# 2InfinityN6eyond/AbsoluteTrack

Hardware: AMD Instinct MI355X
Metric: hand-frames/sec (higher is better)
Workload: dtype f32 (backbone products as two fp16 pieces per operand, fp32 accumulation); 1 GPU; 4 fisheye cameras x 2 hands per frame, 2 views per hand, 96x96 crops, known-skeleton path, full hot path (resample+backbone+head+FK) + all-gather of records; frames_per_gpu=1024, src_image=480x636 u8 x 4 cameras, parallelism=frame-shard x1, world=1, backend=none (single process), outputs_finite=True

## Files before the change

### absolutetrack_amd/csrc/conv_w4.hip

```cpp
#include <type_traits>

#include "ut_kernels.h"
#include "ut_conv_dev.h"

namespace ut {
namespace {

constexpr int W4_WPIX = 288;
constexpr int W4_MI = 9;
constexpr int W4_NLOAD = 9;
constexpr int W4_NSTG = 5;
constexpr int W4_DIST = 2;
constexpr int W4_NSET = W4_DIST + 1;
constexpr unsigned W4_HOOB = 0x80000000u;
static_assert(9 % W4_NSET == 0, "the register sets of the weight fragments line up across slices");
constexpr int w4_cap(int pixels, int wi, int hi) { return ((pixels / (wi * hi)) * (hi + 1) * (wi + 1) + 2 * (wi + 2) + 15) / 16 * 16; }

template <int WI, int HI, int SCH, int WPX, bool S2 = false, bool CHAIN = false>
__global__ __launch_bounds__(256, 1) void conv_w4_kernel(typename std::conditional<CHAIN, W4ChainLaunch, ConvLaunch>::type p, int tiles_n, int n_tiles) {
  extern __shared__ __attribute__((aligned(16))) char smem[];
  constexpr int MI = W4_MI, PW = WI + 1, PH = HI + 1, HW = WI * HI;
  static_assert(!S2 || (SCH == 32 && WPX == 1), "phase planes: two 16-channel planes per buffer, four 32-channel blocks per tile");
  static_assert(!(S2 && CHAIN), "chains: the stride-1 forms");
  constexpr int LDAUX = CHAIN ? 16 : 0;
  constexpr int BM = W4_WPIX * WPX;
  constexpr int NCB = 4 / WPX, BN = 32 * NCB;
  constexpr int NG = SCH / 4, NHG = NG / 2;
  constexpr int KS = 9 * SCH / 16;
  constexpr int NBUF = SCH == 32 ? 2 : 3;
  constexpr int AHEAD = NBUF - 1;
  constexpr int RP = 256 / NG;
  constexpr int CAP = w4_cap(BM, WI, HI);
  constexpr int GSTRIDE = CAP * 16;
  constexpr int STAGE = NG * GSTRIDE;
  constexpr int SLOT = NBUF * STAGE;
  constexpr int KTAB = SLOT + 16;
  constexpr int EPI = SLOT + (CHAIN ? 64 : 16);
  static_assert(BM % HW == 0, "a tile is a whole number of maps: every tile has the same padded layout");
  static_assert(BM * NG == W4_NLOAD * 256 && KS % W4_NSET == 0 && (SCH == 32 || SCH == 16) && (WPX == 1 || WPX == 2), "shape");
  static_assert((NG - 2) * GSTRIDE + (2 * PW + 2) * 16 < 65536, "fragment reads: everything but the lane's base fits the immediate offset");

  const int tid = threadIdx.x;
  const int lane = tid & 63;
  const int wave = __builtin_amdgcn_readfirstlane(tid >> 6);
  const int wm = WPX == 1 ? 0 : wave >> 1;
  const int wco = WPX == 1 ? wave : wave & 1;
  const int fr = lane & 31, fh = lane >> 5;

  const int M = p.n_img * HW;
  int n_slices = (!S2 && p.k_cin > 0 ? p.k_cin : p.cin) / (S2 ? 16 : SCH);
  const int n_chunks = p.k_pad / 32;

  __amdgpu_buffer_rsrc_t a_rsrc = __builtin_amdgcn_make_buffer_rsrc(
      const_cast<float*>(p.in), 0, (int)((size_t)M * (S2 ? 4 : 1) * p.cin * sizeof(float)), 0x00020000);
  __amdgpu_buffer_rsrc_t w_rsrc = __builtin_amdgcn_make_buffer_rsrc(
      const_cast<void*>(p.w_split), 0, (int)((size_t)(p.cout_pad / 32) * n_chunks * 4096), 0x00020000);
  __amdgpu_buffer_rsrc_t r_rsrc = __builtin_amdgcn_make_buffer_rsrc(
      const_cast<float*>(p.res ? p.res : p.bias), 0, p.res ? (int)((size_t)M * p.cout_store * sizeof(float)) : 0, 0x00020000);
  __amdgpu_buffer_rsrc_t o_rsrc =
      __builtin_amdgcn_make_buffer_rsrc(p.out, 0, (int)((size_t)M * p.cout_store * sizeof(float)), 0x00020000);
  const __amdgpu_buffer_rsrc_t q_rsrc = __builtin_amdgcn_make_buffer_rsrc(p.tile_counter, 0, 4, 0x00020000);

  float x_scale = 1.f, x_unscale = 1.f;
  if (p.in_max) {
    bool ok, adapted;
    split_act_scale(p.in_max, p.in_obs, p.split_adaptive, x_scale, x_unscale, ok, adapted);
    split_scale_report(ok, adapted, p.status, p.adapt_count);
  }
  float tot_unscale = p.split_unscale * x_unscale;
  float floor_v = p.relu ? 0.f : -__builtin_huge_valf();
  const float* bias_c = p.bias;
  unsigned* out_max_c = p.out_max;
  int guard_k = 0;
  bool guarded = false;
  float xs_n = x_scale;
  __amdgpu_buffer_rsrc_t a_rsrc_n = a_rsrc, w_rsrc_n = w_rsrc;
  int n_slices_n = n_slices;
  const unsigned row_b = (unsigned)p.cout_store * 4u;

  const int grid = gridDim.x;
  int slot = blockIdx.x;
  if ((grid & 7) == 0) slot = (blockIdx.x & 7) * (grid >> 3) + (blockIdx.x >> 3);

  unsigned h_wa[W4_NLOAD], pb[MI];
#pragma unroll
  for (int j = 0; j < W4_NLOAD; ++j) {
    const int k = RP * j + tid / NG, img = k / HW, rem = k - img * HW, y = rem / WI, x = rem - y * WI;
    h_wa[j] = (unsigned)((PW + 1 + img * (PH * PW) + y * PW + x) * 16 + ((tid % NG) >> 1) * GSTRIDE + (tid & 1) * 8);
  }
#pragma unroll
  for (int i = 0; i < MI; ++i) {
    const int k = wm * W4_WPIX + 32 * i + fr, img = k / HW, rem = k - img * HW, y = rem / WI, x = rem - y * WI;
    pb[i] = (unsigned)((img * (PH * PW) + y * PW + x) * 16 + fh * GSTRIDE);
  }
  const unsigned h_step = (unsigned)(RP * p.cin) * 4u;
#define W4_H_BASE(TILE) ((unsigned)((((TILE) / tiles_n) * BM + tid / NG) * p.cin + 4 * (tid % NG)) * 4u)
#define W4_H_BASE_U(UNIT) ((unsigned)(((UNIT) * BM + tid / NG) * p.cin + 4 * (tid % NG)) * 4u)
  unsigned h_in[S2 ? W4_NLOAD : 1], po_a = 0, po_b = 0, pb1[S2 ? MI : 1];
  if constexpr (S2) {
#pragma unroll
    for (int j = 0; j < W4_NLOAD; ++j) {
      const int k = RP * j + tid / NG, img = k / HW, rem = k - img * HW, y = rem / WI, x = rem - y * WI;
      h_in[j] = (unsigned)(((img * 2 * HI + 2 * y) * 2 * WI + 2 * x) * p.cin + 4 * (tid & 3)) * 4u;
    }
    const bool second = (tid & 4) != 0;
    po_a = second ? 0u : (unsigned)((2 * WI + 1) * p.cin) * 4u;
    po_b = second ? (unsigned)(2 * WI * p.cin) * 4u : (unsigned)p.cin * 4u;
#pragma unroll
    for (int i = 0; i < MI; ++i) pb1[i] = pb[i] + (unsigned)STAGE;
  }
#define W4S_BASE(TILE) ((unsigned)(((TILE) / tiles_n) * (BM * 4)) * (unsigned)p.cin * 4u)

  f32x16 acc[MI];
  u32x4 xp[MI][2];
  u32x4 wf[W4_NSET][2];
  float4 stg[S2 ? W4_NLOAD : W4_NSTG];
  const unsigned w_lane = (unsigned)lane * 16u;

#define W4_READ_X(I, PC, S, TAP, BASE)                                                               \
  xp[I][PC] = *reinterpret_cast<const u32x4*>(smem + (BASE)[I] + (unsigned)(((PC) * NHG + (SCH == 32 ? 2 * (S) : 0)) * GSTRIDE + (((TAP) / 3) * PW + (TAP) % 3) * 16));
#define W4_LOAD_W_OF(RS, SET, PL, CH, S, WROW)                                                       \
  {                                                                                                  \
    const unsigned so_ = (WROW) + (unsigned)((wco * n_chunks + (CH)) * 4096 + ((S) * 2 + (PL)) * 1024); \
    wf[SET][PL] = __builtin_bit_cast(u32x4, __builtin_amdgcn_raw_buffer_load_b128(RS, w_lane, so_, 0)); \
  }
#define W4_LOAD_W(SET, PL, CH, S, WROW) W4_LOAD_W_OF(w_rsrc, SET, PL, CH, S, WROW)
#define W4S_PLANE(Q) ((0x190 >> (Q)) & 1)
#define W4S_TAPP(Q) ((int)((0x414344310ull >> (4 * (Q))) & 15))
#define W4S_TAPO(Q) ((int)((0x715348620ull >> (4 * (Q))) & 15))
#define W4S_BASEOF(Q) ((Q) >= 5 ? pb1 : pb)
#define W4_TAP(Q) (SCH == 32 ? (Q) >> 1 : (Q))
#define W4_CHUNK(SL, Q) (SCH == 32 ? (SL) * 9 + ((Q) >> 1) : ((SL) >> 1) * 9 + (Q))
#define W4_HALF(SL, Q) (SCH == 32 ? (Q) & 1 : (SL) & 1)
#define W4_MFMA(WSET, N)                                                                             \
  {                                                                                                  \
    constexpr int pr_ = (N) / MI, i_ = (N) % MI;                                                     \
    constexpr int wp_ = pr_ == 1 ? 1 : 0, xq_ = pr_ == 0 ? 1 : 0;       \
    acc[i_] = __builtin_amdgcn_mfma_f32_32x32x16_f16(__builtin_bit_cast(f16x8, xp[i_][xq_]),         \
                                                     __builtin_bit_cast(f16x8, wf[WSET][wp_]), acc[i_], 0, 0, 0);  \
  }
#define W4_PIN() { __builtin_amdgcn_sched_barrier(0); asm volatile("" ::: "memory"); __builtin_amdgcn_sched_barrier(0); }
#define W4_ROW_OFF(I, R) ((unsigned)((I) * 32 + 8 * ((R) >> 2) + ((R) & 3)) * row_bs)
#define W4_SPLIT_STORE(V, WA)                                                                        \
  {                                                                                                  \
    unsigned a0_, b0_, a1_, b1_;                                                                     \
    split_pair_scaled((V).x, (V).y, x_scale, a0_, b0_);                                              \
    split_pair_scaled((V).z, (V).w, x_scale, a1_, b1_);                                              \
    *reinterpret_cast<u32x2*>(smem + (WA)) = u32x2{a0_, a1_};                                        \
    *reinterpret_cast<u32x2*>(smem + (WA) + NHG * GSTRIDE) = u32x2{b0_, b1_};                        \
  }

  int tile = slot;
  int next_tile = 0;
  int cur_buf = 0;
  unsigned out_bits = 0;
  const unsigned slot_addr = (unsigned)(unsigned long)(lds_char*)smem + (unsigned)SLOT;
  const int tn_sh = tiles_n == 2 ? 1 : 0, tn_mask = tiles_n - 1;
  int u_c = slot, s_c = 0, u_o = -1, s_o = 0, nx_u = -1, nx_s = 0, adv_u = -1, adv_s = 0, k_c = 0, k_n = 0;
  bool dep = false;
  int steps = 0;
  if constexpr (CHAIN) {
    steps = p.n_layers << tn_sh;
    u_o = grid + slot < n_tiles ? grid + slot : -1;
    if (tid < p.n_layers) {
      const unsigned bits = *p.lay[tid].in_max;
      const int e = (int)(bits >> 23);
      float sc_, un_;
      *reinterpret_cast<int*>(smem + KTAB + 4 * tid) = split_pow2_for(e, bits == 0u || e == 255, sc_, un_);
      if (tid > 0 && e == 255 && blockIdx.x == 0 && p.status) atomicOr(p.status, UT_SPLIT_RANGE);
    }
  }

  for (int k = tid; k < NBUF * STAGE / 16; k += 256) *reinterpret_cast<u32x4*>(smem + k * 16) = u32x4{0, 0, 0, 0};
  __syncthreads();
  unsigned h_base = S2 ? 0u : CHAIN ? W4_H_BASE_U(slot) : W4_H_BASE(tile);
  unsigned w_row = CHAIN ? 0u : (unsigned)((tile % tiles_n) * NCB) * (unsigned)n_chunks * 4096u;
  unsigned w_row_next = w_row;
  if constexpr (CHAIN) k_c = k_n = slot_read(slot_addr + (unsigned)(KTAB - SLOT));
  if constexpr (!S2) {
#pragma unroll
    for (int a = 0; a < AHEAD; ++a)
#pragma unroll
      for (int j = 0; j < W4_NLOAD; ++j) {
        const float4 v = __builtin_bit_cast(float4, __builtin_amdgcn_raw_buffer_load_b128(a_rsrc, h_base + (unsigned)j * h_step, (unsigned)(a * SCH * 4), LDAUX));
        if (a == AHEAD - 1 && KS == 9 && j >= W4_NLOAD - 4) stg[j % W4_NSTG] = v;
        else W4_SPLIT_STORE(v, (unsigned)(a * STAGE) + h_wa[j])
      }
#pragma unroll
    for (int g = 0; g < W4_DIST; ++g) { W4_LOAD_W(g, 0, W4_CHUNK(0, g), W4_HALF(0, g), w_row) W4_LOAD_W(g, 1, W4_CHUNK(0, g), W4_HALF(0, g), w_row) }
  } else {
    const unsigned t0 = W4S_BASE(tile);
#pragma unroll
    for (int j = 0; j < W4_NLOAD; ++j) {
      const float4 v = __builtin_bit_cast(float4, __builtin_amdgcn_raw_buffer_load_b128(a_rsrc, h_in[j] + po_a + t0, 0, 0));
      W4_SPLIT_STORE(v, h_wa[j])
    }
#pragma unroll
    for (int j = 0; j < W4_NLOAD; ++j) {
      const float4 v = __builtin_bit_cast(float4, __builtin_amdgcn_raw_buffer_load_b128(a_rsrc, h_in[j] + po_b + t0, 0, 0));
      if (j == 0) W4_SPLIT_STORE(v, (unsigned)STAGE + h_wa[j])
      else stg[j] = v;
    }
#pragma unroll
    for (int g = 0; g < W4_DIST; ++g) { W4_LOAD_W(g, 0, W4S_TAPO(g), 0, w_row) W4_LOAD_W(g, 1, W4S_TAPO(g), 0, w_row) }
  }
  __syncthreads();
#pragma unroll
  for (int i = 0; i < MI; ++i) {
    W4_READ_X(i, 1, 0, 0, pb)
    if (i < MI - 1) { W4_READ_X(i, 0, 0, 0, pb) }
  }

#define W4_SLOT_BODY(N)                                                                              \
        {                                                                                            \
          if ((N) == 0 && q != KS - 1) { W4_READ_X(MI - 1, 0, W4_HALF(sl, q), W4_TAP(q), rb) }       \
          if ((N) >= 1 && (N) <= 9 && q1 < KS) { W4_READ_X(((N) + 8) % 9, 1, W4_HALF(sl, q1), W4_TAP(q1), rb) } \
          if ((N) >= 1 && (N) <= 9 && q1 == KS) { W4_READ_X(((N) + 8) % 9, 1, 0, 0, nb) }            \
          if ((N) >= 19 && (N) <= 26 && q1 < KS) { W4_READ_X(((N) + 8) % 9, 0, W4_HALF(sl, q1), W4_TAP(q1), rb) } \
          if ((N) >= 19 && (N) <= 26 && q1 == KS) { W4_READ_X(((N) + 8) % 9, 0, 0, 0, nb) }          \
          if (((N) == 10 || (N) == 11) && qd < KS) { W4_LOAD_W(qd % W4_NSET, (N) & 1, W4_CHUNK(sl, qd), W4_HALF(sl, qd), w_row) } \
          if (((N) == 10 || (N) == 11) && qd >= KS) { W4_LOAD_W_OF(wr_after, qd % W4_NSET, (N) & 1, W4_CHUNK(sl_after, qd - KS), W4_HALF(sl_after, qd - KS), row_after) } \
          if ((N) == 12 && q >= 4 && q < 4 + W4_NLOAD) { const float4 v_ = stg[(q + W4_NSTG - 4) % W4_NSTG]; split_pair_scaled(v_.x, v_.y, xs_f, cv0, cv1); } \
          if ((N) == 13 && q >= 4 && q < 4 + W4_NLOAD) {                                             \
            const float4 v_ = stg[(q + W4_NSTG - 4) % W4_NSTG];                                      \
            unsigned a1_, b1_;                                                                       \
            split_pair_scaled(v_.z, v_.w, xs_f, a1_, b1_);                                           \
            *reinterpret_cast<u32x2*>(smem + wbuf + h_wa[(q + 5) % 9]) = u32x2{cv0, a1_};            \
            *reinterpret_cast<u32x2*>(smem + wbuf + h_wa[(q + 5) % 9] + NHG * GSTRIDE) = u32x2{cv1, b1_}; \
          }                                                                                          \
          if (KS == 9 && (N) == 12 && q < 4) { const float4 v_ = stg[q % W4_NSTG]; split_pair_scaled(v_.x, v_.y, xs_p, cv0, cv1); } \
          if (KS == 9 && (N) == 13 && q < 4) {       \
            const float4 v_ = stg[q % W4_NSTG];                                                      \
            unsigned a1_, b1_;                                                                       \
            split_pair_scaled(v_.z, v_.w, xs_p, a1_, b1_);                                           \
            *reinterpret_cast<u32x2*>(smem + pbuf + h_wa[q + 5]) = u32x2{cv0, a1_};                  \
            *reinterpret_cast<u32x2*>(smem + pbuf + h_wa[q + 5] + NHG * GSTRIDE) = u32x2{cv1, b1_};  \
          }                                                                                          \
          if ((N) == 14 && q < W4_NLOAD)                                                             \
            stg[q % W4_NSTG] = __builtin_bit_cast(float4, __builtin_amdgcn_raw_buffer_load_b128(f_rsrc, h_base + (unsigned)q * h_step, f_soff, LDAUX)); \
          if ((N) == 16 && q == KS / 2 && sl == 0 && tid == 0) *reinterpret_cast<int*>(smem + SLOT) = (CHAIN ? 2 * grid : grid) + ticket; \
          W4_PIN();                                                                                  \
          W4_MFMA(ws, N);                                                                            \
          W4_PIN();                                                                                  \
        }
#define W4_SLICE()                                                                                   \
      _Pragma("clang loop unroll(full)") for (int q = 0; q < KS; ++q) {                              \
        const int ws = q % W4_NSET;                                                                  \
        unsigned cv0 = 0, cv1 = 0;      \
         \
        const int q1 = q + 1, qd = q + W4_DIST;                                                      \
        if (q == KS - 1) {                                                                           \
                                       \
          W4_READ_X(MI - 1, 0, W4_HALF(sl, KS - 1), 8, rb)                                           \
                                                                            \
          if (CHAIN && sl == 0) asm volatile("s_waitcnt vmcnt(0)" ::: "memory");                     \
          asm volatile("s_waitcnt lgkmcnt(0)" ::: "memory");                                         \
          __builtin_amdgcn_s_barrier();                                                              \
          asm volatile("" ::: "memory");                                                             \
          if constexpr (CHAIN) {                                                                     \
            if (sl == 0) { W4_CHAIN_NEXT() }                                                         \
          } else if (sl == 0) {                                                                      \
            next_tile = slot_read(slot_addr);                                                        \
            w_row_next = (unsigned)((next_tile % tiles_n) * NCB) * (unsigned)n_chunks * 4096u;       \
          }                                                                                          \
        }                                                                                            \
        W4_SLOT_BODY(0) W4_SLOT_BODY(1) W4_SLOT_BODY(2) W4_SLOT_BODY(3) W4_SLOT_BODY(4) W4_SLOT_BODY(5) W4_SLOT_BODY(6) W4_SLOT_BODY(7) W4_SLOT_BODY(8) \
        W4_SLOT_BODY(9) W4_SLOT_BODY(10) W4_SLOT_BODY(11) W4_SLOT_BODY(12) W4_SLOT_BODY(13) W4_SLOT_BODY(14) W4_SLOT_BODY(15) W4_SLOT_BODY(16) W4_SLOT_BODY(17) \
        W4_SLOT_BODY(18) W4_SLOT_BODY(19) W4_SLOT_BODY(20) W4_SLOT_BODY(21) W4_SLOT_BODY(22) W4_SLOT_BODY(23) W4_SLOT_BODY(24) W4_SLOT_BODY(25) W4_SLOT_BODY(26) \
      }

#define W4S_CV_N(Q) ((Q) == 4 ? 3 : (Q) == 8 ? 1 : 2)
#define W4S_CV_J(Q, NN) ((Q) < 4 ? 2 * (Q) + 1 + (NN) : (Q) == 4 ? (NN) : (Q) < 8 ? 2 * (Q) - 7 + (NN) : 0)
#define W4S_CV_DST(Q) (((Q) < 4 || (Q) == 8) ? (unsigned)STAGE : 0u)
#define W4S_LD_N(Q) ((Q) == 0 ? 3 : (Q) == 4 ? 1 : 2)
#define W4S_LD_J(Q, NN) ((Q) == 0 ? (NN) : (Q) < 4 ? 2 * (Q) + 1 + (NN) : (Q) == 4 ? 0 : 2 * (Q) - 9 + (NN))
#define W4S_SLOT_BODY(N)                                                                             \
        {                                                                                            \
          if ((N) == 0) { W4_READ_X(MI - 1, 0, W4S_PLANE(q), W4S_TAPP(q), W4S_BASEOF(q)) }          \
          if ((N) == 9 && (q == 4 || q == 8)) {                                                      \
                                         \
            asm volatile("s_waitcnt lgkmcnt(0)" ::: "memory");                                       \
            __builtin_amdgcn_s_barrier();                                                            \
            asm volatile("" ::: "memory");                                                           \
            if (q == 8 && sl == 0) {                                                                 \
              next_tile = slot_read(slot_addr);                                                      \
              w_row_next = (unsigned)((next_tile % tiles_n) * NCB) * (unsigned)n_chunks * 4096u;     \
            }                                                                                        \
          }                                                                                          \
          if ((N) >= 1 && (N) <= 9 && q != 4 && q != 8) { W4_READ_X(((N) + 8) % 9, 1, W4S_PLANE(q1), W4S_TAPP(q1), W4S_BASEOF(q1)) } \
          if ((N) >= 10 && (N) <= 18 && (q == 4 || q == 8)) { W4_READ_X(((N) + 8) % 9, 1, W4S_PLANE(q1), W4S_TAPP(q1), W4S_BASEOF(q1)) } \
          if ((N) >= 19 && (N) <= 26) { W4_READ_X(((N) + 8) % 9, 0, W4S_PLANE(q1), W4S_TAPP(q1), W4S_BASEOF(q1)) } \
          if (((N) == 10 || (N) == 11) && qd < 9) { W4_LOAD_W(qd % W4_NSET, (N) & 1, (sl >> 1) * 9 + W4S_TAPO(qd), sl & 1, w_row) } \
          if (((N) == 10 || (N) == 11) && qd >= 9) { W4_LOAD_W(qd % W4_NSET, (N) & 1, (sl_after >> 1) * 9 + W4S_TAPO(qd - 9), sl_after & 1, row_after) } \
           \
          if ((N) >= 10 && (N) <= 21 && ((N) - 10) / 4 < W4S_CV_N(q)) {                              \
            const float4 v_ = stg[W4S_CV_J(q, ((N) - 10) / 4) % 9];                                  \
            constexpr int part_ = ((N) - 10) & 3;                                                    \
            if (part_ == 0 || part_ == 2) {                                                          \
              const f16x2 h_ = __builtin_bit_cast(f16x2, __builtin_amdgcn_cvt_pkrtz((part_ ? v_.z : v_.x) * x_scale, (part_ ? v_.w : v_.y) * x_scale)); \
              (part_ ? cvh1 : cvh0) = __builtin_bit_cast(unsigned, h_);                              \
              cvf = (float)h_[0];                                                                    \
            } else {                                                                                 \
              const f16x2 h_ = __builtin_bit_cast(f16x2, part_ == 1 ? cvh0 : cvh1);                  \
              const float ra_ = __builtin_fmaf(part_ == 1 ? v_.x : v_.z, x_scale, -cvf);             \
              const float rb_ = __builtin_fmaf(part_ == 1 ? v_.y : v_.w, x_scale, -(float)h_[1]);    \
              const unsigned p_ = __builtin_bit_cast(unsigned, __builtin_amdgcn_cvt_pkrtz(ra_, rb_)); \
              if (part_ == 1) cvp0 = p_;                                                             \
              else {                                                                                 \
                *reinterpret_cast<u32x2*>(smem + W4S_CV_DST(q) + h_wa[W4S_CV_J(q, ((N) - 10) / 4) % 9]) = u32x2{cvh0, cvh1}; \
                *reinterpret_cast<u32x2*>(smem + W4S_CV_DST(q) + h_wa[W4S_CV_J(q, ((N) - 10) / 4) % 9] + NHG * GSTRIDE) = u32x2{cvp0, p_}; \
              }                                                                                      \
            }                                                                                        \
          }                                                                                          \
          if ((N) >= 22 && (N) <= 24 && (N) - 22 < W4S_LD_N(q))                                      \
            stg[W4S_LD_J(q, (N) - 22) % 9] = __builtin_bit_cast(float4, __builtin_amdgcn_raw_buffer_load_b128(    \
                a_rsrc, h_in[W4S_LD_J(q, (N) - 22) % 9] + (q < 4 ? hb_a : hb_b), f_soff, 0));        \
          if ((N) == 16 && q == 1 && sl == 0 && tid == 0) *reinterpret_cast<int*>(smem + SLOT) = grid + ticket; \
          W4_PIN();                                                                                  \
          W4_MFMA(ws, N);                                                                            \
          W4_PIN();                                                                                  \
        }
#define W4S_SLICE()                                                                                  \
      _Pragma("clang loop unroll(full)") for (int q = 0; q < 9; ++q) {                               \
        const int ws = q % W4_NSET;                                                                  \
        unsigned cvh0 = 0, cvh1 = 0, cvp0 = 0;                       \
        float cvf = 0.f;                                                                             \
        const int q1 = (q + 1) % 9, qd = q + W4_DIST;                                                \
        W4S_SLOT_BODY(0) W4S_SLOT_BODY(1) W4S_SLOT_BODY(2) W4S_SLOT_BODY(3) W4S_SLOT_BODY(4) W4S_SLOT_BODY(5) W4S_SLOT_BODY(6) W4S_SLOT_BODY(7) W4S_SLOT_BODY(8) \
        W4S_SLOT_BODY(9) W4S_SLOT_BODY(10) W4S_SLOT_BODY(11) W4S_SLOT_BODY(12) W4S_SLOT_BODY(13) W4S_SLOT_BODY(14) W4S_SLOT_BODY(15) W4S_SLOT_BODY(16) W4S_SLOT_BODY(17) \
        W4S_SLOT_BODY(18) W4S_SLOT_BODY(19) W4S_SLOT_BODY(20) W4S_SLOT_BODY(21) W4S_SLOT_BODY(22) W4S_SLOT_BODY(23) W4S_SLOT_BODY(24) W4S_SLOT_BODY(25) W4S_SLOT_BODY(26) \
      }

#define W4_CHAIN_NEXT()                                                                              \
  {                                                                                                  \
    const int l_c = s_c >> tn_sh;                                                                    \
    const bool fresh = s_c + 1 == steps, two = u_o >= 0;                                             \
    adv_s = fresh ? 0 : s_c + 1;                                                                     \
    nx_s = two ? s_o : adv_s;                                                                        \
    const int l_n = nx_s >> tn_sh, l_g = l_c + 1 < p.n_layers ? l_c + 1 : l_c;                       \
    int tk_, kn_, kg_;                                                                               \
    asm volatile("ds_read_b32 %0, %3\n\tds_read_b32 %1, %4\n\tds_read_b32 %2, %5\n\ts_waitcnt lgkmcnt(0)" \
                 : "=&v"(tk_), "=&v"(kn_), "=&v"(kg_)                                                \
                 : "v"(slot_addr), "v"(slot_addr + (unsigned)(KTAB - SLOT + 4 * l_n)), "v"(slot_addr + (unsigned)(KTAB - SLOT + 4 * l_g)) : "memory"); \
    const int tk = __builtin_amdgcn_readfirstlane(tk_);                                              \
    adv_u = fresh ? ((unsigned)tk < (unsigned)n_tiles ? tk : -1) : u_c;                              \
    nx_u = two ? u_o : adv_u;                                                                        \
    dep = !two && !fresh && (adv_s & tn_mask) == 0;                                                  \
    guarded = l_c + 1 < p.n_layers;                                                                  \
    guard_k = __builtin_amdgcn_readfirstlane(kg_);                                                   \
    const unsigned o_bytes = (unsigned)M * (unsigned)p.cout_store * 4u;                              \
    {                                                                                                \
      const W4Layer& lc = p.lay[l_c];                                                                \
      r_rsrc = __builtin_amdgcn_make_buffer_rsrc(const_cast<float*>(lc.res ? lc.res : lc.bias), 0, lc.res ? (int)o_bytes : 0, 0x00020000); \
      o_rsrc = __builtin_amdgcn_make_buffer_rsrc(lc.out, 0, (int)o_bytes, 0x00020000);               \
      bias_c = lc.bias;                                                                              \
      out_max_c = lc.out_max;                                                                        \
      tot_unscale = lc.split_unscale * __uint_as_float((unsigned)(127 - k_c) << 23);                 \
      floor_v = lc.relu ? 0.f : -__builtin_huge_valf();                                              \
      bb4 = *reinterpret_cast<const float4*>(bias_c + (s_c & tn_mask) * BN + wco * 32 + 4 * (lane & 7)); \
    }                                                                                                \
    if (nx_u >= 0) {                                                                                 \
      const W4Layer& ln = p.lay[l_n];                                                                \
      a_rsrc_n = __builtin_amdgcn_make_buffer_rsrc(const_cast<float*>(ln.in), 0, (int)((unsigned)M * (unsigned)p.cin * 4u), 0x00020000); \
      w_rsrc_n = __builtin_amdgcn_make_buffer_rsrc(const_cast<void*>(ln.w_split), 0, (int)((size_t)(p.cout_pad / 32) * n_chunks * 4096), 0x00020000); \
      k_n = __builtin_amdgcn_readfirstlane(kn_);                                                     \
      xs_n = __uint_as_float((unsigned)(127 + k_n) << 23);                                           \
      n_slices_n = (ln.k_cin > 0 ? ln.k_cin : p.cin) / SCH;                                          \
      w_row_next = (unsigned)((nx_s & tn_mask) * NCB) * (unsigned)n_chunks * 4096u;                  \
    }                                                                                                \
  }

  for (;;) {
    int ticket = 0;
    if (tid == 0 && (!CHAIN || s_c + 1 == steps)) ticket = __builtin_amdgcn_raw_ptr_buffer_atomic_add_i32(1, q_rsrc, 0, 0, 0);
    if constexpr (CHAIN) out_bits = 0;
#pragma unroll
    for (int i = 0; i < MI; ++i)
#pragma unroll
      for (int e = 0; e < 16; ++e) acc[i][e] = 0.f;

    float4 bb4 = float4{0.f, 0.f, 0.f, 0.f};
    if constexpr (!CHAIN) bb4 = *reinterpret_cast<const float4*>(p.bias + (tile % tiles_n) * BN + wco * 32 + 4 * (lane & 7));
    if constexpr (S2) {
      for (int sl = 0; sl < n_slices; ++sl) {
        const bool last_slice = sl == n_slices - 1;
        const unsigned f_soff = last_slice ? 0u : (unsigned)(sl + 1) * 64u;
        const unsigned f_tb = W4S_BASE(last_slice ? next_tile : tile);
        const unsigned hb_a = po_a + f_tb, hb_b = po_b + f_tb;
        const int sl_after = last_slice ? 0 : sl + 1;
        const unsigned row_after = last_slice ? w_row_next : w_row;
        W4S_SLICE()
      }
    } else
    for (int sl = 0; sl < n_slices; ++sl) {
      const bool last_slice = sl == n_slices - 1;
      const int b1 = cur_buf + 1 == NBUF ? 0 : cur_buf + 1, b2 = b1 + 1 == NBUF ? 0 : b1 + 1;
      unsigned rbuf = (unsigned)__builtin_amdgcn_readfirstlane(cur_buf * STAGE), nbuf = (unsigned)__builtin_amdgcn_readfirstlane(b1 * STAGE);
      unsigned wbuf = (unsigned)__builtin_amdgcn_readfirstlane((NBUF == 2 ? b1 : b2) * STAGE), pbuf = nbuf;
      asm volatile("" : "+s"(rbuf), "+s"(nbuf), "+s"(wbuf), "+s"(pbuf));
      const int f_sl = sl + AHEAD < n_slices ? sl + AHEAD : sl + AHEAD - n_slices;
      if constexpr (CHAIN) {
        if (sl + AHEAD == n_slices) h_base = nx_u >= 0 && !dep ? W4_H_BASE_U(nx_u) : W4_HOOB;
      } else if (sl + AHEAD == n_slices) h_base = W4_H_BASE(next_tile);
      const unsigned f_soff = (unsigned)f_sl * (SCH * 4);
      const int sl_after = last_slice ? 0 : sl + 1;
      const unsigned row_after = last_slice ? w_row_next : w_row;
      const bool f_next = CHAIN && sl + AHEAD >= n_slices, p_next = CHAIN && sl > 0 && sl - 1 + AHEAD >= n_slices;
      const float xs_f = f_next ? xs_n : x_scale, xs_p = p_next ? xs_n : x_scale;
      const __amdgpu_buffer_rsrc_t f_rsrc = f_next ? a_rsrc_n : a_rsrc, wr_after = CHAIN && last_slice ? w_rsrc_n : w_rsrc;
      unsigned rb[MI], nb[MI];
#pragma unroll
      for (int i = 0; i < MI; ++i) { rb[i] = pb[i] + rbuf; nb[i] = pb[i] + nbuf; }
      W4_SLICE()
      cur_buf = b1;
    }
    {
      const int tm = CHAIN ? u_c : tile / tiles_n, tn = CHAIN ? s_c & tn_mask : tile - tm * tiles_n;
      const bool ragged = tm * BM + BM > M;
      const int ch = tn * BN + wco * 32 + fr;
      const float bb = bias_c[ch];
      const unsigned base = ch < p.cout_store ? (unsigned)((tm * BM + wm * W4_WPIX + 4 * fh) * p.cout_store + ch) * 4u : W4_HOOB;
      const unsigned keep_n = base != W4_HOOB ? 0x7FFFFFFFu : 0u;
      if (!ragged) {
        unsigned row_bs = (unsigned)__builtin_amdgcn_readfirstlane((int)row_b);
        asm volatile("" : "+s"(row_bs));
        const int ch4 = tn * BN + wco * 32 + 4 * (lane & 7);
        const unsigned base4 = ch4 < p.cout_store ? (unsigned)((tm * BM + wm * W4_WPIX + (lane >> 3)) * p.cout_store + ch4) * 4u : W4_HOOB;
        const unsigned keep4 = base4 != W4_HOOB ? 0x7FFFFFFFu : 0u;
        float4 rr[S2 ? 1 : 6][4];
        if constexpr (!S2) {
#pragma unroll
          for (int i = 0; i < 5; ++i)
#pragma unroll
            for (int t = 0; t < 4; ++t)
              rr[i][t] = __builtin_bit_cast(float4, __builtin_amdgcn_raw_buffer_load_b128(r_rsrc, base4, (unsigned)(32 * i + 8 * t) * row_bs, LDAUX));
        }
        char* const ex = smem + EPI + wave * 4096;
#define W4_EX_WRITE(H)                                                                               \
        _Pragma("unroll") for (int r = 0; r < 8; ++r)                                                \
          *reinterpret_cast<float*>(ex + ((H) & 1) * 2048 + (8 * (r >> 2) + 4 * fh + (r & 3)) * 128 + fr * 4) = acc[(H) >> 1][8 * ((H) & 1) + r];
        W4_EX_WRITE(0)
#pragma unroll
        for (int h = 0; h < 2 * MI; ++h) {
          const int i = h >> 1;
          if (!S2 && (h & 1) == 0 && i + 5 < MI) {
#pragma unroll
            for (int t = 0; t < 4; ++t)
              rr[(i + 5) % 6][t] = __builtin_bit_cast(float4, __builtin_amdgcn_raw_buffer_load_b128(r_rsrc, base4, (unsigned)(32 * (i + 5) + 8 * t) * row_bs, LDAUX));
          }
          if (h + 1 < 2 * MI) { W4_EX_WRITE(h + 1) }
#pragma unroll
          for (int t2 = 0; t2 < 2; ++t2) {
            const int t = 2 * (h & 1) + t2;
            const float4 a = *reinterpret_cast<const float4*>(ex + (h & 1) * 2048 + (8 * t2 + (lane >> 3)) * 128 + (lane & 7) * 16);
            const float4 res = S2 ? float4{0.f, 0.f, 0.f, 0.f} : rr[S2 ? 0 : i % 6][t];
            u32x4 o;
            o.x = __float_as_uint(fmaxf(fmaf(a.x, tot_unscale, bb4.x + res.x), floor_v));
            o.y = __float_as_uint(fmaxf(fmaf(a.y, tot_unscale, bb4.y + res.y), floor_v));
            o.z = __float_as_uint(fmaxf(fmaf(a.z, tot_unscale, bb4.z + res.z), floor_v));
            o.w = __float_as_uint(fmaxf(fmaf(a.w, tot_unscale, bb4.w + res.w), floor_v));
            unsigned mk;
            asm volatile("v_max3_u32 %0, %2, %3, %4\n\tv_max_u32 %0, %0, %5\n\tv_and_b32 %0, %0, %6\n\tv_max_u32 %1, %1, %0"
                         : "=&v"(mk), "+v"(out_bits) : "v"(o.x), "v"(o.y), "v"(o.z), "v"(o.w), "v"(keep4));
            __builtin_amdgcn_raw_buffer_store_b128(o, o_rsrc, base4, (unsigned)(32 * i + 8 * t) * row_bs, 0);
          }
        }
#undef W4_EX_WRITE
      } else {
#pragma unroll
        for (int i = 0; i < MI; ++i) {
          float r1[16];
          unsigned off = base + (unsigned)(i * 32) * row_b;
#pragma unroll
          for (int r = 0; r < 16; ++r) {
            r1[r] = __uint_as_float(__builtin_amdgcn_raw_buffer_load_b32(r_rsrc, off, 0, LDAUX));
            off += ((r & 3) == 3 ? 5u : 1u) * row_b;
          }
          off = base + (unsigned)(i * 32) * row_b;
#pragma unroll
          for (int r = 0; r < 16; ++r) {
            const unsigned o = __float_as_uint(fmaxf(fmaf(acc[i][r], tot_unscale, bb + r1[r]), floor_v));
            const int pix = wm * W4_WPIX + i * 32 + 8 * (r >> 2) + 4 * fh + (r & 3);
            out_bits = max(out_bits, o & (tm * BM + pix < M ? keep_n : 0u));
            __builtin_amdgcn_raw_buffer_store_b32(o, o_rsrc, off, 0, 0);
            off += ((r & 3) == 3 ? 5u : 1u) * row_b;
          }
        }
      }
    }
    if constexpr (CHAIN) {
      {
        unsigned wb = out_bits;
#pragma unroll
        for (int o = 32; o; o >>= 1) {
          const unsigned other = (unsigned)__shfl_xor((int)wb, o);
          wb = other > wb ? other : wb;
        }
        if (lane == 0) {
          if (out_max_c && wb > __hip_atomic_load(out_max_c, __ATOMIC_RELAXED, __HIP_MEMORY_SCOPE_AGENT)) atomicMax(out_max_c, wb);
          const int eo = (int)(wb >> 23);
          if (guarded && (eo == 255 || eo + guard_k > 142) && p.status) atomicOr(p.status, UT_SPLIT_RANGE);
        }
      }
      if (nx_u < 0) break;
      const bool two = u_o >= 0;
      u_c = nx_u; s_c = nx_s;
      if (two) { u_o = adv_u; s_o = adv_s; }
      a_rsrc = a_rsrc_n; w_rsrc = w_rsrc_n; x_scale = xs_n; k_c = k_n; n_slices = n_slices_n;
      w_row = w_row_next;
      if (dep) {
        asm volatile("s_waitcnt vmcnt(0)" ::: "memory");
        __syncthreads();
        h_base = W4_H_BASE_U(u_c);
        int bo = cur_buf;
#pragma unroll
        for (int a = 0; a < AHEAD; ++a) {
          const unsigned dst = (unsigned)__builtin_amdgcn_readfirstlane(bo * STAGE);
#pragma unroll
          for (int j = 0; j < W4_NLOAD; ++j) {
            const float4 v = __builtin_bit_cast(float4, __builtin_amdgcn_raw_buffer_load_b128(a_rsrc, h_base + (unsigned)j * h_step, (unsigned)(a * SCH * 4), LDAUX));
            if (a == AHEAD - 1 && KS == 9 && j >= W4_NLOAD - 4) stg[j % W4_NSTG] = v;
            else W4_SPLIT_STORE(v, dst + h_wa[j])
          }
          bo = bo + 1 == NBUF ? 0 : bo + 1;
        }
        __syncthreads();
        const unsigned rb0 = (unsigned)__builtin_amdgcn_readfirstlane(cur_buf * STAGE);
        unsigned rb[MI];
#pragma unroll
        for (int i = 0; i < MI; ++i) rb[i] = pb[i] + rb0;
#pragma unroll
        for (int i = 0; i < MI; ++i) {
          W4_READ_X(i, 1, 0, 0, rb)
          if (i < MI - 1) { W4_READ_X(i, 0, 0, 0, rb) }
        }
      }
    } else {
      if ((unsigned)next_tile >= (unsigned)n_tiles) break;
      tile = next_tile;
      w_row = w_row_next;
    }
  }
  if constexpr (!CHAIN) { if (p.out_max) publish_abs_max(p.out_max, out_bits); }
#undef W4_H_BASE
#undef W4_H_BASE_U
#undef W4_LOAD_W_OF
#undef W4_CHAIN_NEXT
#undef W4_READ_X
#undef W4_LOAD_W
#undef W4_TAP
#undef W4_CHUNK
#undef W4_HALF
#undef W4_MFMA
#undef W4_PIN
#undef W4_ROW_OFF
#undef W4_SPLIT_STORE
#undef W4_SLOT_BODY
#undef W4_SLICE
#undef W4S_PLANE
#undef W4S_TAPP
#undef W4S_TAPO
#undef W4S_BASEOF
#undef W4S_BASE
#undef W4S_CV_N
#undef W4S_CV_J
#undef W4S_CV_DST
#undef W4S_LD_N
#undef W4S_LD_J
#undef W4S_SLOT_BODY
#undef W4S_SLICE
}

template <int WI, int HI, int SCH, int WPX, bool S2 = false>
hipError_t launch_w4_cfg(const ConvLaunch& c, hipStream_t s) {
  constexpr int BM = W4_WPIX * WPX, BN = 128 / WPX;
  const long M = (long)c.n_img * c.Ho * c.Wo;
  const int tiles_m = (int)((M + BM - 1) / BM), tiles_n = c.cout_store / BN;
  const int n_tiles = tiles_m * tiles_n;
  constexpr int lds = (SCH == 32 ? 2 : 3) * (SCH / 4) * w4_cap(BM, WI, HI) * 16 + 16 + 4 * 4096;
  return launch_with_lds<&conv_w4_kernel<WI, HI, SCH, WPX, S2>>(c.device, lds, persistent_grid(c.num_cu, n_tiles), 256, s, c, tiles_n, n_tiles);
}

template <int WI, int HI, int SCH, int WPX>
hipError_t launch_w4_chain_cfg(const W4ChainLaunch& c, hipStream_t s) {
  constexpr int BM = W4_WPIX * WPX, BN = 128 / WPX;
  const long M = (long)c.n_img * c.Ho * c.Wo;
  const int units = (int)((M + BM - 1) / BM), tiles_n = c.cout_store / BN;
  constexpr int lds = (SCH == 32 ? 2 : 3) * (SCH / 4) * w4_cap(BM, WI, HI) * 16 + 64 + 4 * 4096;
  return launch_with_lds<&conv_w4_kernel<WI, HI, SCH, WPX, false, true>>(c.device, lds, persistent_grid(c.num_cu, units), 256, s, c, tiles_n, units);
}

}

W4Form conv_w4_form(const ConvLaunch& c) {
  const bool common = c.w_split && c.split_unscale > 0.f && c.ksize == 3 && c.pad == 1 && c.cslice == 32 &&
                      c.cin % 32 == 0 && c.cout_pad >= c.cout_store && !c.out_nchw && c.splits == 0 &&
                      c.k_pad == 9 * c.cin && c.tile_counter && c.num_cu > 0 &&
                      offsets_fit_32(c.n_img, c.H, c.W, c.cin) && offsets_fit_32(c.n_img, c.Ho, c.Wo, c.cout_store);
  if (!common) return W4_NONE;
  if (c.stride == 2)
    return c.cin >= 64  && c.cout_store % 128 == 0 && c.H == 2 * c.Ho && c.W == 2 * c.Wo && !c.res &&
           ((c.Wo == 12 && c.Ho == 12) || (c.Wo == 6 && c.Ho == 6)) ? W4_STRIDE2 : W4_NONE;
  if (c.stride != 1 || c.cin < 64 || c.H != c.Ho || c.W != c.Wo) return W4_NONE;
  if (c.k_cin != 0 && (c.k_cin % 32 != 0 || c.k_cin < 64 || c.k_cin > c.cin)) return W4_NONE;
  if (c.cout_store % 128 == 0) return (c.W == 12 && c.H == 12) || (c.W == 6 && c.H == 6) ? W4_TILES128 : W4_NONE;
  return c.cout_store == 64 && c.W == 24 && c.H == 24 ? W4_MAP24 : W4_NONE;
}

hipError_t launch_conv_w4(const ConvLaunch& c, hipStream_t s) {
  const W4Form form = conv_w4_form(c);
  if (form == W4_NONE) return hipErrorInvalidValue;
  if (form == W4_STRIDE2) return c.Wo == 12 ? launch_w4_cfg<12, 12, 32, 1, true>(c, s) : launch_w4_cfg<6, 6, 32, 1, true>(c, s);
  if (form == W4_MAP24) return launch_w4_cfg<24, 24, 16, 2>(c, s);
  return c.W == 12 ? launch_w4_cfg<12, 12, 32, 1>(c, s) : launch_w4_cfg<6, 6, 32, 1>(c, s);
}


bool conv_w4_chainable(const ConvLaunch& a, const ConvLaunch& b) {
  const W4Form fa = conv_w4_form(a), fb = conv_w4_form(b);
  if (fa != fb || (fa != W4_TILES128 && fa != W4_MAP24)) return false;
  if (a.cout_store > 256 || a.cin != a.cout_store) return false;
  return b.in == a.out && b.in_obs == a.out_max && a.out_max && b.in_max && a.in_max && !a.split_adaptive && !b.split_adaptive &&
         a.n_img == b.n_img && a.H == b.H && a.W == b.W && a.cin == b.cin && a.cout_store == b.cout_store && a.cout_pad == b.cout_pad &&
         a.k_pad == b.k_pad && a.status == b.status && a.device == b.device && a.num_cu == b.num_cu;
}

bool conv_w4_chain_fills(const ConvLaunch& c) {
  const long units = ((long)c.n_img * c.Ho * c.Wo + W4_WPIX - 1) / W4_WPIX;
  return c.cout_store <= 128 || units >= (long)c.num_cu;
}

hipError_t launch_conv_w4_chain(const ConvLaunch* layers, int n_layers, hipStream_t s) {
  if (n_layers < 1 || n_layers > W4_MAX_CHAIN) return hipErrorInvalidValue;
  for (int l = 1; l < n_layers; ++l)
    if (!conv_w4_chainable(layers[l - 1], layers[l])) return hipErrorInvalidValue;
  const W4Form form = conv_w4_form(layers[0]);
  if ((form != W4_TILES128 && form != W4_MAP24) || !layers[0].in_max || !layers[0].out_max) return hipErrorInvalidValue;
  W4ChainLaunch c{};
  static_cast<ConvLaunch&>(c) = layers[0];
  c.n_layers = n_layers;
  for (int l = 0; l < n_layers; ++l) {
    const ConvLaunch& a = layers[l];
    c.lay[l] = W4Layer{a.in, a.res, a.out, a.w_split, a.bias, a.in_max, a.out_max, a.split_unscale, a.k_cin, a.relu};
  }
  if (form == W4_MAP24) return launch_w4_chain_cfg<24, 24, 16, 2>(c, s);
  return c.W == 12 ? launch_w4_chain_cfg<12, 12, 32, 1>(c, s) : launch_w4_chain_cfg<6, 6, 32, 1>(c, s);
}

}
```

Measured before the change: 168,600 hand-frames/s.

## Overlap chained conv epilogue with last-slice MFMA tail

For chained 32-channel convolutions, the last K-slice now runs its second half as a special tail loop. That loop interleaves the epilogue of each finished accumulator block with the remaining MFMAs: LDS transpose, residual loads, bias/ReLU, the max tracking and the stores. It also prefetches the next tile's weights and staged inputs, which hides epilogue latency behind matrix work. The cost is many more live registers and a complex hand-scheduled path. The path only applies to whole tiles; ragged tiles fall back to the normal path.

```diff
diff --git a/absolutetrack_amd/csrc/conv_w4.hip b/absolutetrack_amd/csrc/conv_w4.hip
--- a/absolutetrack_amd/csrc/conv_w4.hip
+++ b/absolutetrack_amd/csrc/conv_w4.hip
@@ -14,6 +14,7 @@
 constexpr int W4_NSET = W4_DIST + 1;
 constexpr unsigned W4_HOOB = 0x80000000u;
 static_assert(9 % W4_NSET == 0, "the register sets of the weight fragments line up across slices");
+constexpr int W4_TAIL = 9;
 constexpr int w4_cap(int pixels, int wi, int hi) { return ((pixels / (wi * hi)) * (hi + 1) * (wi + 1) + 2 * (wi + 2) + 15) / 16 * 16; }
 
 template <int WI, int HI, int SCH, int WPX, bool S2 = false, bool CHAIN = false>
@@ -35,6 +36,9 @@
   constexpr int STAGE = NG * GSTRIDE;
   constexpr int SLOT = NBUF * STAGE;
   constexpr int KTAB = SLOT + 16;
+  constexpr bool TAIL = CHAIN && SCH == 32;
+  constexpr int KH = KS - W4_TAIL;
+  static_assert(!TAIL || (KH == 9 && W4_TAIL >= W4_DIST + 1), "tail: the second half of an 18-step slice");
   constexpr int EPI = SLOT + (CHAIN ? 64 : 16);
   static_assert(BM % HW == 0, "a tile is a whole number of maps: every tile has the same padded layout");
   static_assert(BM * NG == W4_NLOAD * 256 && KS % W4_NSET == 0 && (SCH == 32 || SCH == 16) && (WPX == 1 || WPX == 2), "shape");
@@ -114,6 +118,8 @@
   f32x16 acc[MI];
   u32x4 xp[MI][2];
   u32x4 wf[W4_NSET][2];
+  u32x4 wt[TAIL ? W4_TAIL - W4_DIST : 1][2];
+  u32x4 xt[TAIL ? 3 : 1][2];
   float4 stg[S2 ? W4_NLOAD : W4_NSTG];
   const unsigned w_lane = (unsigned)lane * 16u;
 
@@ -125,6 +131,13 @@
     wf[SET][PL] = __builtin_bit_cast(u32x4, __builtin_amdgcn_raw_buffer_load_b128(RS, w_lane, so_, 0)); \
   }
 #define W4_LOAD_W(SET, PL, CH, S, WROW) W4_LOAD_W_OF(w_rsrc, SET, PL, CH, S, WROW)
+#define W4_LOAD_WT(SET, PL, CH, S)                                                                   \
+  {                                                                                                  \
+    const unsigned so_ = w_row + (unsigned)((wco * n_chunks + (CH)) * 4096 + ((S) * 2 + (PL)) * 1024); \
+    wt[SET][PL] = __builtin_bit_cast(u32x4, __builtin_amdgcn_raw_buffer_load_b128(w_rsrc, w_lane, so_, 0)); \
+  }
+#define W4_READ_XT(SET, I, PC, S, TAP, BASE)                                                         \
+  xt[SET][PC] = *reinterpret_cast<const u32x4*>(smem + (BASE)[I] + (unsigned)(((PC) * NHG + 2 * (S)) * GSTRIDE + (((TAP) / 3) * PW + (TAP) % 3) * 16));
 #define W4S_PLANE(Q) ((0x190 >> (Q)) & 1)
 #define W4S_TAPP(Q) ((int)((0x414344310ull >> (4 * (Q))) & 15))
 #define W4S_TAPO(Q) ((int)((0x715348620ull >> (4 * (Q))) & 15))
@@ -239,12 +252,21 @@
           if ((N) == 14 && q < W4_NLOAD)                                                             \
             stg[q % W4_NSTG] = __builtin_bit_cast(float4, __builtin_amdgcn_raw_buffer_load_b128(f_rsrc, h_base + (unsigned)q * h_step, f_soff, LDAUX)); \
           if ((N) == 16 && q == KS / 2 && sl == 0 && tid == 0) *reinterpret_cast<int*>(smem + SLOT) = (CHAIN ? 2 * grid : grid) + ticket; \
+          if constexpr (TAIL) {       \
+            if (tl && ((N) == 15 || (N) == 17) && q >= W4_DIST) { W4_LOAD_WT(q - W4_DIST, (N) == 17 ? 1 : 0, W4_CHUNK(sl, KH + q), W4_HALF(sl, KH + q)) } \
+            if (tl && q == KH - 1 && (N) == 16) { W4_READ_XT(1, 0, 1, W4_HALF(sl, KH + 1), W4_TAP(KH + 1), rb) } \
+            if (tl && q == KH - 1 && (N) == 18) { W4_READ_XT(1, 0, 0, W4_HALF(sl, KH + 1), W4_TAP(KH + 1), rb) } \
+            if (tl && q == KH - 1 && (N) >= 19)                                                      \
+              rr3[((N) - 19) / 4 % 3][((N) - 19) % 4] = __builtin_bit_cast(float4, __builtin_amdgcn_raw_buffer_load_b128(r_rsrc, t_base4, (unsigned)(8 * ((N) - 19)) * t_row_bs, LDAUX)); \
+          }                                                                                          \
           W4_PIN();                                                                                  \
           W4_MFMA(ws, N);                                                                            \
           W4_PIN();                                                                                  \
         }
-#define W4_SLICE()                                                                                   \
-      _Pragma("clang loop unroll(full)") for (int q = 0; q < KS; ++q) {                              \
+#define W4_SLICE() W4_SLICE_N(KS, false)
+#define W4_SLICE_N(KQ, TL)                                                                           \
+      _Pragma("clang loop unroll(full)") for (int q = 0; q < (KQ); ++q) {                            \
+        const bool tl = (TL);                                                                        \
         const int ws = q % W4_NSET;                                                                  \
         unsigned cv0 = 0, cv1 = 0;      \
          \
@@ -391,7 +413,16 @@
         const unsigned row_after = last_slice ? w_row_next : w_row;
         W4S_SLICE()
       }
-    } else
+    } else {
+    const bool t_whole = TAIL && u_c * BM + BM <= M;
+    unsigned t_row_bs = 0u, t_base4 = W4_HOOB, t_keep4 = 0u;
+    float4 rr3[3][4];
+    if constexpr (TAIL) {
+      t_row_bs = (unsigned)__builtin_amdgcn_readfirstlane((int)row_b);
+      asm volatile("" : "+s"(t_row_bs));
+      const int ch4 = (s_c & tn_mask) * BN + wco * 32 + 4 * (lane & 7);
+      if (ch4 < p.cout_store) { t_base4 = (unsigned)((u_c * BM + wm * W4_WPIX + (lane >> 3)) * p.cout_store + ch4) * 4u; t_keep4 = 0x7FFFFFFFu; }
+    }
     for (int sl = 0; sl < n_slices; ++sl) {
       const bool last_slice = sl == n_slices - 1;
       const int b1 = cur_buf + 1 == NBUF ? 0 : cur_buf + 1, b2 = b1 + 1 == NBUF ? 0 : b1 + 1;
@@ -411,8 +442,103 @@
       unsigned rb[MI], nb[MI];
 #pragma unroll
       for (int i = 0; i < MI; ++i) { rb[i] = pb[i] + rbuf; nb[i] = pb[i] + nbuf; }
-      W4_SLICE()
+      bool tailed = false;
+      if constexpr (TAIL) {
+        if (last_slice && t_whole) {
+          W4_SLICE_N(KH, true)
+          char* const ex = smem + EPI + wave * 4096;
+          float4 ea[4];
+          u32x4 eo[4];
+          u32x4 wn[W4_DIST][2];
+          const auto comp = [](const float4& v, int c) { return c == 0 ? v.x : c == 1 ? v.y : c == 2 ? v.z : v.w; };
+#define W4_TAIL_VALUE(O, A, RES)                                                                     \
+          (O) = __float_as_uint(fmaxf(fmaf((A), tot_unscale, (RES)), floor_v));
+#define W4_TAIL_WORD(O)                                                                              \
+          {                                                                                          \
+            unsigned mk;                                                                             \
+            asm volatile("v_max3_u32 %0, %2, %3, %4\n\tv_max_u32 %0, %0, %5\n\tv_and_b32 %0, %0, %6\n\tv_max_u32 %1, %1, %0" \
+                         : "=&v"(mk), "+v"(out_bits) : "v"((O).x), "v"((O).y), "v"((O).z), "v"((O).w), "v"(t_keep4)); \
+          }
+#pragma unroll
+          for (int i = 0; i < MI; ++i) {
+            unsigned cv0 = 0, cv1 = 0;
+#pragma unroll
+            for (int s = 0; s < 3 * W4_TAIL; ++s) {
+              const int j = s / 3, pr = s % 3, g = W4_TAIL * i + j, g2 = g + 2, i2 = g2 < MI * W4_TAIL ? g2 / W4_TAIL : 0, k2 = KH + g2 % W4_TAIL;
+              const int e = i > 0 ? i - 1 : 0, i_r = i + 2 < MI ? i + 2 : 0;
+              if (pr < 2 && g2 < MI * W4_TAIL && g2 % W4_TAIL != 0) { W4_READ_XT(g2 % 3, i2, 1 - pr, W4_HALF(sl, k2), W4_TAP(k2), rb) }
+              if (i == 0 && s == 2) { W4_READ_X(MI - 1, 0, W4_HALF(sl, KH), W4_TAP(KH), rb) }
+              if (i > 0 && s >= 2 && s <= 5) {
+#pragma unroll
+                for (int r = 4 * (s - 2); r < 4 * (s - 2) + 4; ++r)
+                  *reinterpret_cast<float*>(ex + (8 * (r >> 2) + 4 * fh + (r & 3)) * 128 + fr * 4) = acc[e][r & 15];
+              }
+              if (i > 0 && (s == 7 || s == 8)) {
+#pragma unroll
+                for (int t = 2 * (s - 7); t < 2 * (s - 7) + 2; ++t)
+                  ea[t & 3] = *reinterpret_cast<const float4*>(ex + (8 * (t & 3) + (lane >> 3)) * 128 + (lane & 7) * 16);
+              }
+              if (s >= 10 && s <= 25) {
+                const int t = (s - 10) >> 2, c = (s - 10) & 3;
+                if (i > 0) { W4_TAIL_VALUE(eo[t][c], comp(ea[t], c), comp(bb4, c) + comp(rr3[e % 3][t], c)) }
+                if (i > 0 && c == 3) { W4_TAIL_WORD(eo[t]) }
+                if (i + 2 < MI && c == 3)
+                  rr3[i_r % 3][t] = __builtin_bit_cast(float4, __builtin_amdgcn_raw_buffer_load_b128(r_rsrc, t_base4, (unsigned)(32 * i_r + 8 * t) * t_row_bs, LDAUX));
+                if (i > 0 && c == 3) __builtin_amdgcn_raw_buffer_store_b128(eo[t], o_rsrc, t_base4, (unsigned)(32 * e + 8 * t) * t_row_bs, 0);
+              }
+              if (i == 0 && s >= 23) {
+                const unsigned so_ = row_after + (unsigned)((wco * n_chunks + W4_CHUNK(0, (s - 23) >> 1)) * 4096 + (W4_HALF(0, (s - 23) >> 1) * 2 + ((s - 23) & 1)) * 1024);
+                wn[((s - 23) >> 1) % W4_DIST][(s - 23) & 1] = __builtin_bit_cast(u32x4, __builtin_amdgcn_raw_buffer_load_b128(wr_after, w_lane, so_, 0));
+              }
+              if (i < 4 && s == 8) { const float4 v_ = stg[i & 3]; split_pair_scaled(v_.x, v_.y, xs_f, cv0, cv1); }
+              if (i < 4 && s == 9) {
+                const float4 v_ = stg[i & 3];
+                unsigned a1_, b1_;
+                split_pair_scaled(v_.z, v_.w, xs_f, a1_, b1_);
+                *reinterpret_cast<u32x2*>(smem + wbuf + h_wa[5 + (i & 3)]) = u32x2{cv0, a1_};
+                *reinterpret_cast<u32x2*>(smem + wbuf + h_wa[5 + (i & 3)] + NHG * GSTRIDE) = u32x2{cv1, b1_};
+              }
+              W4_PIN();
+              {
+                const u32x4 xa = j == 0 ? xp[i][pr == 0 ? 1 : 0] : xt[g % 3][pr == 0 ? 1 : 0];
+                const u32x4 wa = j < W4_DIST ? wf[(KH + j) % W4_NSET][pr == 1 ? 1 : 0] : wt[j < W4_DIST ? 0 : j - W4_DIST][pr == 1 ? 1 : 0];
+                acc[i] = __builtin_amdgcn_mfma_f32_32x32x16_f16(__builtin_bit_cast(f16x8, xa), __builtin_bit_cast(f16x8, wa), acc[i], 0, 0, 0);
+              }
+              W4_PIN();
+            }
+          }
+          asm volatile("s_waitcnt lgkmcnt(0)" ::: "memory");
+          __builtin_amdgcn_s_barrier();
+          asm volatile("" ::: "memory");
+#pragma unroll
+          for (int g = 0; g < W4_DIST; ++g) { wf[g][0] = wn[g][0]; wf[g][1] = wn[g][1]; }
+#pragma unroll
+          for (int i = 0; i < MI; ++i) {
+            W4_READ_X(i, 1, 0, 0, nb)
+            if (i < MI - 1) { W4_READ_X(i, 0, 0, 0, nb) }
+          }
+#pragma unroll
+          for (int r = 0; r < 16; ++r) *reinterpret_cast<float*>(ex + (8 * (r >> 2) + 4 * fh + (r & 3)) * 128 + fr * 4) = acc[MI - 1][r];
+#pragma unroll
+          for (int t = 0; t < 4; ++t) {
+            const float4 a = *reinterpret_cast<const float4*>(ex + (8 * t + (lane >> 3)) * 128 + (lane & 7) * 16);
+            const float4 res = rr3[(MI - 1) % 3][t];
+            u32x4 o;
+            W4_TAIL_VALUE(o.x, a.x, bb4.x + res.x)
+            W4_TAIL_VALUE(o.y, a.y, bb4.y + res.y)
+            W4_TAIL_VALUE(o.z, a.z, bb4.z + res.z)
+            W4_TAIL_VALUE(o.w, a.w, bb4.w + res.w)
+            W4_TAIL_WORD(o)
+            __builtin_amdgcn_raw_buffer_store_b128(o, o_rsrc, t_base4, (unsigned)(32 * (MI - 1) + 8 * t) * t_row_bs, 0);
+          }
+#undef W4_TAIL_VALUE
+#undef W4_TAIL_WORD
+          tailed = true;
+        }
+      }
+      if (!tailed) { W4_SLICE() }
       cur_buf = b1;
+    }
     }
     {
       const int tm = CHAIN ? u_c : tile / tiles_n, tn = CHAIN ? s_c & tn_mask : tile - tm * tiles_n;
@@ -422,6 +548,7 @@
       const unsigned base = ch < p.cout_store ? (unsigned)((tm * BM + wm * W4_WPIX + 4 * fh) * p.cout_store + ch) * 4u : W4_HOOB;
       const unsigned keep_n = base != W4_HOOB ? 0x7FFFFFFFu : 0u;
       if (!ragged) {
+        if constexpr (!TAIL) {
         unsigned row_bs = (unsigned)__builtin_amdgcn_readfirstlane((int)row_b);
         asm volatile("" : "+s"(row_bs));
         const int ch4 = tn * BN + wco * 32 + 4 * (lane & 7);
@@ -466,6 +593,7 @@
           }
         }
 #undef W4_EX_WRITE
+        }
       } else {
 #pragma unroll
         for (int i = 0; i < MI; ++i) {
@@ -557,6 +685,9 @@
 #undef W4_SPLIT_STORE
 #undef W4_SLOT_BODY
 #undef W4_SLICE
+#undef W4_SLICE_N
+#undef W4_LOAD_WT
+#undef W4_READ_XT
 #undef W4S_PLANE
 #undef W4S_TAPP
 #undef W4S_TAPO
```

Result: no change. 169,700 hand-frames/s (median of 6 runs) (+0.6%).
